# PIC4SeR/nav2_social_mpc_controller

Measured on AMD Instinct MI355X. Metric: MPC solves/sec (horizon=18, 8 agents, max 40 LM iterations, Ceres termination rules), higher is better.
Workload: dtype f64; 1 GPU; BASELINE configs[2] per GPU: batch=8192 scenes/GPU, 8 people, horizon=18 (T=28, block=6, P=6, M=226), 200x200 u8 costmap per scene, DENSE_SCHUR, max 40 LM iterations with Ceres termination rules; consecutive steps overlapped on 4 HIP streams, every stream on a scene batch of its own; scenes_per_gpu=8192, people=8, T=28, P=6, M=226, streams=4, distinct_scene_batches=4

## Files before the change

### nav2_social_mpc_controller_amd/csrc/smpc_launch.hpp

```cpp
#pragma once

#include <hip/hip_runtime.h>
#include <stdint.h>

#include "../../include/smpc.h"
#include "smpc_math.hpp"

namespace smpc {

constexpr int kWave = 64;
constexpr double kNoTarget = 1e300;
constexpr int kSoc = 15;

typedef double v4d __attribute__((ext_vector_type(4)));
typedef double v2d __attribute__((ext_vector_type(2)));

struct KParams {
  int B, T, N, CH, bl, nb, P, nbounded, nfeas;
  int size_x, size_y, costmap_shared;
  double dt, resolution;
  double inv_resolution;
  smpc_params prm;
  const double* pose0;
  const double* init_params;
  const double* path_pts;
  const double* goal_yaw;
  const double* people;
  const uint8_t* has_people;
  const int32_t* T_scene;
  const uint8_t* costmap;
  const double* costmap_origin;
  double* o_params;
  double* o_cmds;
  double* o_path;
  int32_t* o_status;
  int32_t* o_reason;
  int32_t* o_iterations;
  int32_t* o_evaluations;
  double* o_initial_cost;
  double* o_final_cost;
  int* queue;
  const double* people_rec;
  const double* people_aux;
  const int32_t* order;
  int hp_A;
  int full_gram;
  int prio_step;
  int lone_help;
  double* stage_rec;
  double* stage_aux;
  unsigned long long* stamps;
  const double* e_x;
  double* e_residuals;
  double* e_jacobian;
  double* e_cost;
  double* e_gradient;
  int e_M;
  int e_row_order;
  MathTab mt;
  AtanNodeTab an;
  const smpc_scene_params* scene_params;
  double* o_trace;
  int32_t* o_trace_n;
  int trace_rows;
  int stage_at_fetch;
};
constexpr int kTraceCols = SMPC_TRACE_COLS;
constexpr int kQueueWords = 4;

__host__ __device__ constexpr bool lone_trip_kernel(int W, bool vt, bool sp, bool trace) { return W == 32 && !vt && !sp && !trace; }

typedef const KParams __attribute__((address_space(4))) * KParamsK;

constexpr int kSensInRegsMaxBlocks = 6;
__host__ __device__ constexpr int eval_extra_doubles(int T, int P, int W) {
  return (64 / W) * (2 * T * P) + (P / 2 > kSensInRegsMaxBlocks ? (64 / W) * (5 * (P / 2) * W) : 0);
}
__host__ __device__ constexpr int atan_tab_offset(int slot_doubles, int extra_doubles) { return (slot_doubles + extra_doubles + 3) & ~3; }
constexpr int kAtanTabDoubles = kAtanNodes * kAtanNodeStride;
constexpr int kGramChunk = 16;
__host__ __device__ constexpr int gram_red_doubles(int W) { return W * (kGramChunk + 1); }
__host__ __device__ constexpr int wave_extra_doubles(int P, int W) {
  return (kWave / W) * ((P / 2 > 1 ? P / 2 - 1 : 1) * (P + 1));
}

struct LdsLayout {
  int ag;
  int valid;
  int cs;
  int inc;
  int cst;
  int stepst;
  int part;
  int hz;
  int sp;
  int lanec;
  int lm;
  int gram;
  int scratch;
  int total;
};
// ... 88 lines not shown
```

### nav2_social_mpc_controller_amd/csrc/smpc_lm.hpp

```cpp
#pragma once

#include <hip/hip_runtime.h>

#include "smpc_math.hpp"

namespace smpc {

#ifdef SMPC_STAMPS
__device__ unsigned long long g_ls_dbg[8];
#define SMPC_LS_COUNT(i, n) do { if ((threadIdx.x & 31) == 0) atomicAdd(&g_ls_dbg[i], (unsigned long long)(n)); } while (0)
#else
#define SMPC_LS_COUNT(i, n) do { } while (0)
#endif


__device__ inline void fullpiv_solve(double* A, double* b, int* perm, double* z, double* out, int n) {
  for (int i = 0; i < n; ++i) perm[i] = i;
  for (int kk = 0; kk < n; ++kk) {
    int pr = kk, pc = kk;
    double best = -1.0;
    for (int i = kk; i < n; ++i)
      for (int j = kk; j < n; ++j) {
        const double v = fabs(A[i * n + j]);
        if (v > best) { best = v; pr = i; pc = j; }
// ... 325 lines not shown
  for (int i = 0; i < 4; ++i) {
    const double rt = roots[i];
    const bool in = rt >= lo && rt <= hi;
    if (__any(in)) { const double v = eval_poly_reg<nc>(poly, rt); if (in && v < opt_v) { opt_v = v; opt_x = rt; } }
  }
  const double sx[3] = {lower.x, current.x, previous.x};
#pragma unroll
  for (int smp = 0; smp < 3; ++smp) {
    const bool in = sx[smp] >= lo && sx[smp] <= hi;
    if (__any(in)) { const double v = eval_poly_reg<nc>(poly, sx[smp]); if (in && v < opt_v) { opt_v = v; opt_x = sx[smp]; } }
  }
  step_size = opt_x;
  return true;
}

__device__ inline double clampd(double v, double lo, double hi) { return (v != v) ? v : fmin(fmax(v, lo), hi); }

__device__ inline double yaw_roundtrip(double yaw) {
  double sz, cz;
  sincos(yaw * 0.5, &sz, &cz);
  return atan2(2.0 * (cz * sz), cz * cz - sz * sz);
}


__device__ inline bool armijo_holds(double value, double cost, double gd0, double alpha) {
  return isfinite(value) && !(value > fma(1e-4 * gd0, alpha, cost));
}

enum Phase { PH_FETCH = 0, PH_INIT = 1, PH_LS = 2, PH_REEVAL = 3, PH_DONE = 4, PH_IDLE = 5 };

enum Scal { S_COST = 0, S_XNORM, S_GMAX, S_RADIUS, S_DECF, S_MCC, S_GD0, S_DIRMAX, S_PREV_X, S_PREV_V, S_PREV_G,
            S_CUR_X, S_CUR_V, S_CUR_G, S_INITIAL_COST, S_FIRST_V, S_COUNT };

struct LmRegs {
  int phase, iter, evals, num_invalid, ls_iters, n_samples, status, reason;
  bool step_successful, at_least_one, prev_vv, prev_gv, cur_vv, cur_gv, first_vv;
};

}
```

### nav2_social_mpc_controller_amd/csrc/smpc_solve_body.inc

```
  static_assert(!kSP || kVT, "a kernel with per-scene weights and bounds reads its horizon per scene as well");
  static_assert(!kTrace || (kVT && kSP), "the trace is compiled for the most general variant only");
  const auto& k = *(KParamsK)__builtin_amdgcn_kernarg_segment_ptr();
  constexpr int P = 2 * NB;
  constexpr int S = kWave / W;
  constexpr bool kLone = lone_trip_kernel(W, kVT, kSP, kTrace);
  extern __shared__ __attribute__((aligned(32))) double lds_all[];
  const int lane = threadIdx.x & 63;
  Ctx c;
  c.kp = &k;
  c.L = make_layout(Shape::T(k), Shape::N(k), P, kLayoutSolve, W, kSP);
  c.ag = k.people_rec;
  {
    double* atab = lds_all + atan_tab_offset(S * c.L.total, wave_extra_doubles(P, W));
    load_atan_nodes(c.kp, atab, lane);
    c.atab = atab;
  }
  const auto& prm = k.prm;
  const int T = Shape::T(k);
  int slot, q, qc;
  bool act;
  double *Hs, *Lw, *gs, *gu, *xc, *xt, *dl, *sc, *bc, *rs, *sv, *scratch;
  int32_t* rw;
  auto bind = [&](int lane_t) {
    slot = lane_t / W;
    c.sl = lane_t - slot * W;
    c.slot = slot;
    c.lds = lds_all + (size_t)slot * c.L.total;
    c.wave_lds = lds_all + (size_t)S * c.L.total;
    Hs = c.lds + c.L.lm;
    gs = Hs + P * P;
    gu = gs + P;
    xc = gu + P;
    xt = xc + P;
    dl = xt + P;
    sc = dl + P;
    sv = sc + P;
    rw = reinterpret_cast<int32_t*>(sv + S_COUNT);
    Lw = c.lds + c.L.cs;
    bc = Lw + P * P;
    rs = bc + 4 * P;
    scratch = rs + 3 * P;
    q = c.sl;
    act = q < P;
    qc = act ? q : 0;
  };
  bind(lane);
  auto slot_any = [&](bool pred) -> bool {
    const unsigned long long slot_bits = (W == 64) ? ~0ull : (0xffffffffull << (32 * slot));
    return (__ballot(pred) & slot_bits) != 0ull;
  };
  auto reduce3 = [&](double a, double b, double m, double& sa, double& sb, double& sm) {
    double* w3 = rs;
    if (act) { w3[q] = a; w3[P + q] = b; w3[2 * P + q] = m; }
    wave_lds_fence();
    sa = 0.0; sb = 0.0; sm = 0.0;
#pragma unroll
    for (int i = 0; i < P; ++i) { sa += w3[i]; sb += w3[P + i]; sm = fmax(sm, w3[2 * P + i]); }
  };

  auto trace_row = [&](int row, double cost, double cost_change, double gmax, double step_norm, double rho, double radius,
                       int ls_evals, bool accepted) {
    const auto& kt = *c.kp;
    if (row >= kt.trace_rows || c.sl >= kTraceCols) return;
    const int j = c.sl;
    const double v = j == 0 ? (double)row : j == 1 ? cost : j == 2 ? cost_change : j == 3 ? gmax : j == 4 ? step_norm
                   : j == 5 ? rho : j == 6 ? radius : j == 7 ? (double)ls_evals : (accepted ? 1.0 : 0.0);
    kt.o_trace[((size_t)c.scene * kt.trace_rows + row) * kTraceCols + j] = v;
  };

  LmRegs R;
  R.phase = PH_FETCH;
  R.iter = R.evals = R.num_invalid = R.ls_iters = R.n_samples = 0;
  R.status = SMPC_NO_CONVERGENCE; R.reason = SMPC_REASON_MAX_ITERATIONS;
  R.step_successful = R.at_least_one = R.prev_vv = R.prev_gv = R.cur_vv = R.cur_gv = R.first_vv = false;
  auto park = [&]() {
    rw[0] = R.iter; rw[1] = R.evals; rw[2] = R.num_invalid; rw[3] = R.ls_iters; rw[4] = R.n_samples; rw[5] = R.status;
    rw[6] = R.reason;
    rw[7] = (R.step_successful ? 1 : 0) | (R.at_least_one ? 2 : 0) | (R.prev_vv ? 4 : 0) | (R.prev_gv ? 8 : 0) |
            (R.cur_vv ? 16 : 0) | (R.cur_gv ? 32 : 0) | (R.first_vv ? 64 : 0);
  };
  auto unpark = [&]() {
    R.iter = rw[0]; R.evals = rw[1]; R.num_invalid = rw[2]; R.ls_iters = rw[3]; R.n_samples = rw[4]; R.status = rw[5];
    R.reason = rw[6];
    const int f = rw[7];
    R.step_successful = f & 1; R.at_least_one = f & 2; R.prev_vv = f & 4; R.prev_gv = f & 8;
    R.cur_vv = f & 16; R.cur_gv = f & 32; R.first_vv = f & 64;
  };
  bool ever_loaded = false;
  if constexpr (kLone) *reinterpret_cast<unsigned long long*>(rw + 8) = 0ull;
#ifdef SMPC_STAMPS
  for (int i = 0; i < 8; ++i) c.acc[i] = 0;
  for (int i = 0; i < 4; ++i) c.acc2[i] = 0;
  c.t_last = __builtin_amdgcn_s_memtime();
#endif

  for (;;) {
    SMPC_STAMP(c, 6);
    {
      KParamsK kp_t = c.kp;
      asm volatile("" : "+s"(kp_t));
      c.kp = kp_t;
    }
    const auto& k = *c.kp;
    const auto& prm = k.prm;
    const int T = Shape::T(k);
    if constexpr (!Shape::kFixed) c.L = make_layout(Shape::T(k), Shape::N(k), P, kLayoutSolve, W, kSP);
    {
      int lane_t = lane;
      asm volatile("" : "+v"(lane_t));
      bind(lane_t);
    }
    if (R.phase == PH_FETCH) {
      int scene = 0;
      if (c.sl == 0) {
        scene = atomicAdd(k.queue, 1);
        if (k.order) {
          while (scene < k.B) {
            const int want = k.order[scene];
            if (want >= 0 && want < k.B) { scene = want; break; }
            scene = atomicAdd(k.queue, 1);
          }
        }
      }
      scene = __shfl(scene, slot * W, 64);
      if (scene < k.B) {
        load_scene<W, kVT, kSP, Shape, Shape::kStageAtFetch>(c, scene);
        ever_loaded = true;
        wave_lds_fence();
        const Horizon hz0 = get_horizon<NB, kVT, Shape>(c);
        double v = 0.0;
        if (act && (q >> 1) <= hz0.blast) {
          const bool bnd = (q >> 1) < hz0.nbounded;
          const double lo0 = bnd ? ((q & 1) ? SMPC_SCENE_PRM(c, kSP, prm, w_min) : SMPC_SCENE_PRM(c, kSP, prm, v_min)) : -1.7976931348623157e308;
          const double hi0 = bnd ? ((q & 1) ? SMPC_SCENE_PRM(c, kSP, prm, w_max) : SMPC_SCENE_PRM(c, kSP, prm, v_max)) : 1.7976931348623157e308;
          v = clampd(k.init_params[(size_t)scene * P + q] + 0.0, lo0, hi0);
        }
        if (act) { xc[q] = v; xt[q] = v; }
        double xn, u0, u1;
        reduce3(v * v, 0.0, 0.0, xn, u0, u1);
        sv[S_XNORM] = fast_sqrt(xn);
        R.phase = PH_INIT;
        R.iter = 0; R.evals = 0; R.num_invalid = 0;
        R.status = SMPC_NO_CONVERGENCE; R.reason = SMPC_REASON_MAX_ITERATIONS;
        R.step_successful = true; R.at_least_one = false;
      } else {
        if (!ever_loaded) {
          load_scene<W, kVT, kSP, Shape, Shape::kStageAtFetch>(c, 0, false);
          ever_loaded = true;
          if (act) xt[q] = 0.0;
        }
        R.phase = PH_IDLE;
      }
    }
    if (__all(R.phase == PH_IDLE)) break;
    SMPC_STAMP(c, 0);
    if constexpr (kLone) {
      const bool idle = R.phase == PH_IDLE;
      const unsigned long long ib = __ballot(idle);
      const bool half = ((ib ^ (ib >> 32)) & 1ull) != 0ull;
      const bool lone = half && k.lone_help != 0 && Shape::N(k) >= 2 && __ballot(!idle && c.has_people) != 0ull;
      *trip_mode(c) = !lone ? kTripPaired : idle ? kTripHelper : kTripOwner;
      *reinterpret_cast<unsigned long long*>(rw + 8) += 1ull + (half ? 1ull << 21 : 0ull) + (lone ? 1ull << 42 : 0ull);
    }
    if (k.prio_step > 0) {
      const int mine = (R.phase == PH_IDLE) ? 0 : R.evals;
      int age = __builtin_amdgcn_readfirstlane(mine);
      if (S == 2) age = max(age, __builtin_amdgcn_readlane(mine, 32));
      const int step = k.prio_step;
      if (age >= 3 * step) __builtin_amdgcn_s_setprio(3);
      else if (age >= 2 * step) __builtin_amdgcn_s_setprio(2);
      else if (age >= step) __builtin_amdgcn_s_setprio(1);
      else __builtin_amdgcn_s_setprio(0);
    }

    park();
    const int phase_at_sweep = R.phase;
    auto need_rest = [&]() -> bool {
      if (phase_at_sweep != PH_LS) return phase_at_sweep != PH_IDLE;
      if (k.full_gram) return true;
      const double* gt = c.lds + c.L.gram;
      const double* svp = c.lds + c.L.lm + P * P + 6 * P;
      const unsigned long long slot_bits = (W == 64) ? ~0ull : (0xffffffffull << (32 * c.slot));
      const bool col_finite = (__ballot(c.sl <= P && !isfinite(gt[min(c.sl, P) * (P + 1) + P])) & slot_bits) == 0ull;
      return !col_finite || armijo_holds(0.5 * gt[P * (P + 1) + P], svp[S_COST], svp[S_GD0], svp[S_CUR_X]);
    };
    sweep<NB, W, false, kVT, kSP, Shape, kLone>(c, xt, nullptr, nullptr, need_rest);
    {
      int lane_t = lane;
      asm volatile("" : "+v"(lane_t));
      bind(lane_t);
    }
    GramView GH;
    GH.base = c.lds + c.L.gram;
    GH.ld = P + 1;
    unpark();
    const Horizon hz = get_horizon<NB, kVT, Shape>(c);
    const bool bounded = act && (q >> 1) < hz.nbounded;
    const double lo_q = bounded ? ((q & 1) ? SMPC_SCENE_PRM(c, kSP, prm, w_min) : SMPC_SCENE_PRM(c, kSP, prm, v_min)) : -1.7976931348623157e308;
    const double hi_q = bounded ? ((q & 1) ? SMPC_SCENE_PRM(c, kSP, prm, w_max) : SMPC_SCENE_PRM(c, kSP, prm, v_max)) : 1.7976931348623157e308;
    const bool gram_full = c.gram_full;
    const bool finite = !gram_full || !slot_any(c.sl <= P && !isfinite(GH.base[min(c.sl, P) * GH.ld + min(c.sl, P)]));
    const double val = 0.5 * GH(P, P);
    bool new_iteration = false;

    auto adopt_trial_point = [&]() {
      double xa = 0.0, gm = 0.0;
      if (act) {
        xa = xt[q];
        xc[q] = xa;
        const double scq = sc[q];
        const double* grow = GH.base + q * GH.ld;
#pragma unroll
        for (int b = 0; b < P; ++b) Hs[q * P + b] = grow[b] * scq * sc[b];
        const double g = grow[P];
        gu[q] = g; gs[q] = g * scq;
        gm = fabs(xa - clampd(xa - g, lo_q, hi_q));
      }
      double xn, u0, gmax;
      reduce3(xa * xa, 0.0, gm, xn, u0, gmax);
      sv[S_XNORM] = fast_sqrt(xn);
      sv[S_GMAX] = gmax;
    };
    auto candidate = [&]() {
      const double cost = sv[S_COST];
      const double cand_cost = R.cur_vv ? sv[S_CUR_V] : 1.7976931348623157e308;
      const double d = act ? xc[q] - xt[q] : 0.0;
      double sn2, u0, u1;
      reduce3(d * d, 0.0, 0.0, sn2, u0, u1);
      const double step_norm = fast_sqrt(sn2);
      const bool tol_allowed = !prm.fixed_iterations && (!prm.tol_needs_successful_step || R.at_least_one);
      if (tol_allowed && step_norm <= prm.param_tol * (sv[S_XNORM] + prm.param_tol)) {
        if constexpr (kTrace) trace_row(R.iter, cost, cost - cand_cost, sv[S_GMAX], step_norm, 0.0, sv[S_RADIUS], R.n_samples, false);
        R.status = SMPC_CONVERGENCE; R.reason = SMPC_REASON_PARAMETER_TOL; R.phase = PH_DONE; return;
      }
      const double cost_change = cost - cand_cost;
      if (tol_allowed && fabs(cost_change) <= prm.fn_tol * cost) {
        if constexpr (kTrace) trace_row(R.iter, cost, cost_change, sv[S_GMAX], step_norm, 0.0, sv[S_RADIUS], R.n_samples, false);
        R.status = SMPC_CONVERGENCE; R.reason = SMPC_REASON_FUNCTION_TOL; R.phase = PH_DONE; return;
      }
      const double rho = (cand_cost >= 1.7976931348623157e308) ? -1.7976931348623157e308 : div_fast(cost_change, sv[S_MCC]);
      if (rho > 1e-3 && !gram_full) {
        R.phase = PH_REEVAL;
        return;
      }
      if (rho > 1e-3) {
        adopt_trial_point();
        sv[S_COST] = cand_cost;
        R.step_successful = true; R.at_least_one = true;
        const double t = 2.0 * rho - 1.0;
        sv[S_RADIUS] = fmin(1e16, div_fast(sv[S_RADIUS], fmax(1.0 / 3.0, 1.0 - t * t * t)));
        sv[S_DECF] = 2.0;
      } else {
        sv[S_RADIUS] = sv[S_RADIUS] / sv[S_DECF];
        sv[S_DECF] *= 2.0;
      }
      if constexpr (kTrace) {
        trace_row(R.iter, sv[S_COST], cost_change, sv[S_GMAX], step_norm, rho, sv[S_RADIUS], R.n_samples, R.step_successful);
      }
      new_iteration = true;
    };

    if (R.phase == PH_INIT) {
      ++R.evals;
      sv[S_COST] = val;
      sv[S_INITIAL_COST] = val;
      if (kVT && reinterpret_cast<const int*>(c.lds + c.L.hz)[6] != 0) {
        R.status = SMPC_FAILURE; R.reason = SMPC_REASON_SHORT_PATH; R.phase = PH_DONE;
      } else if (!finite) {
        R.status = SMPC_FAILURE; R.reason = SMPC_REASON_EVAL_FAILED; R.phase = PH_DONE;
      } else {
        if (act) sc[q] = 1.0 / (1.0 + sqrt(GH.base[q * GH.ld + q]));
        wave_lds_fence();
        adopt_trial_point();
        sv[S_RADIUS] = 1e4; sv[S_DECF] = 2.0;
        if constexpr (kTrace) trace_row(0, val, 0.0, sv[S_GMAX], 0.0, 0.0, 1e4, 0, true);
        new_iteration = true;
      }
    } else if (R.phase == PH_LS) {
      ++R.evals;
      const double dq = act ? dl[q] : 0.0;
      double gd, u0, u1;
      reduce3(act ? dq * GH.base[q * GH.ld + P] : 0.0, 0.0, 0.0, gd, u0, u1);
      R.cur_vv = finite && isfinite(val);
      R.cur_gv = R.cur_vv && isfinite(gd);
      sv[S_CUR_V] = val; sv[S_CUR_G] = gd;
      const double alpha = sv[S_CUR_X];
      if (R.n_samples == 1) { sv[S_FIRST_V] = val; R.first_vv = R.cur_vv; }
      if (R.cur_vv && armijo_holds(val, sv[S_COST], sv[S_GD0], alpha)) {
        if (act) dl[q] = dq * alpha;
        candidate();
      } else {
        ++R.ls_iters;
        bool failed = R.ls_iters >= 20;
        double step_size = 0.0;
        if (!failed) {
          Sample lower{0.0, sv[S_COST], sv[S_GD0], true, true};
          Sample previous{sv[S_PREV_X], sv[S_PREV_V], sv[S_PREV_G], R.prev_vv, R.prev_gv};
          Sample current{alpha, val, gd, R.cur_vv, R.cur_gv};
          SMPC_STAMP(c, 6);
          if (!interpolate_step_fast(lower, previous, current, 1e-3 * alpha, 0.6 * alpha, step_size))
          { SMPC_LS_COUNT(7, 1); step_size = interpolate_step(lower, previous, current, 1e-3 * alpha, 0.6 * alpha, scratch); }
          SMPC_STAMP(c, 7);
          failed = step_size * sv[S_DIRMAX] < 1e-9;
        }
        if (!failed) {
          sv[S_PREV_X] = alpha; sv[S_PREV_V] = val; sv[S_PREV_G] = gd; R.prev_vv = R.cur_vv; R.prev_gv = R.cur_gv;
          sv[S_CUR_X] = step_size;
          if (act) xt[q] = clampd(xc[q] + step_size * dq, lo_q, hi_q);
          ++R.n_samples;
        } else if (R.n_samples > 1) {
          if (act) xt[q] = clampd(xc[q] + dq, lo_q, hi_q);
          const double v1 = R.first_vv ? sv[S_FIRST_V] : 1.7976931348623157e308;
          const bool would_accept = R.first_vv && ((sv[S_COST] - v1) / sv[S_MCC] > 1e-3);
          if (would_accept) {
            R.phase = PH_REEVAL;
          } else {
            R.cur_vv = R.first_vv;
            sv[S_CUR_V] = v1;
            wave_lds_fence();
            candidate();
          }
        } else {
          candidate();
        }
      }
    } else if (R.phase == PH_REEVAL) {
      ++R.evals;
      R.cur_vv = finite && isfinite(val);
      sv[S_CUR_V] = val;
      candidate();
    }

    if (new_iteration) {
      for (;;) {
        if (R.iter >= prm.max_iterations) { R.status = SMPC_NO_CONVERGENCE; R.reason = SMPC_REASON_MAX_ITERATIONS; R.phase = PH_DONE; break; }
        if (R.step_successful && sv[S_GMAX] <= prm.gradient_tol && !prm.fixed_iterations) { R.status = SMPC_CONVERGENCE; R.reason = SMPC_REASON_GRADIENT_TOL; R.phase = PH_DONE; break; }
        if (sv[S_RADIUS] <= 1e-32) { R.status = SMPC_CONVERGENCE; R.reason = SMPC_REASON_MIN_RADIUS; R.phase = PH_DONE; break; }
        ++R.iter;
        R.step_successful = false;
        int ql = q;
        asm volatile("" : "+v"(ql));
        const double radius = sv[S_RADIUS];
        const double inv_radius = div_fast(1.0, radius);
        double arow[P], Lr[P], invd[P];
#pragma unroll
        for (int j = 0; j < P; ++j) arow[j] = Hs[qc * P + j];
        const double gsq = act ? gs[q] : 0.0;
        const double d2 = clampd(Hs[qc * P + qc], 1e-6, 1e32) * inv_radius;
        bool ok = true;
#pragma unroll
        for (int j = 0; j < P; ++j) {
          double s_ = arow[j] + ((j == ql) ? d2 : 0.0);
#pragma unroll
          for (int kk = 0; kk < j; ++kk) s_ = fma(-Lr[kk], Lw[j * P + kk], s_);
          if (ql == j) bc[j] = s_;
          wave_lds_fence();
          const double dpiv = bc[j];
          ok = ok && (dpiv > 0.0) && isfinite(dpiv);
          const double inv = rsqrt_pos(fmax(dpiv, 1e-300));
          invd[j] = inv;
          Lr[j] = s_ * inv;
          if (act && ql > j) Lw[q * P + j] = Lr[j];
          wave_lds_fence();
        }
        double accf = gsq, yq = 0.0;
#pragma unroll
        for (int kk = 0; kk < P; ++kk) {
          const double yk_own = accf * invd[kk];
          if (ql == kk) { bc[P + kk] = yk_own; yq = yk_own; }
          wave_lds_fence();
          const double yk = bc[P + kk];
          accf = fma((ql > kk) ? -Lr[kk] : 0.0, yk, accf);
        }
        double accb = yq, zq = 0.0;
#pragma unroll
        for (int kk = P - 1; kk >= 0; --kk) {
          const double zk_own = accb * invd[kk];
          if (ql == kk) { bc[2 * P + kk] = zk_own; zq = zk_own; }
          wave_lds_fence();
          const double zk = bc[2 * P + kk];
          accb = fma((act && ql < kk) ? -Lw[kk * P + qc] : 0.0, zk, accb);
        }
        const double stepq = act ? -zq : 0.0;
        bool valid = ok && !slot_any(act && !isfinite(stepq));
        double mcc = 0.0;
        if (valid) {
          if (act) bc[3 * P + q] = stepq;
          wave_lds_fence();
          double rowv = 0.0;
#pragma unroll
          for (int b = 0; b < P; ++b) rowv = fma(arow[b], bc[3 * P + b], rowv);
          double sg, sHs, u1;
          reduce3(stepq * gsq, act ? stepq * rowv : 0.0, 0.0, sg, sHs, u1);
          mcc = -sg - 0.5 * sHs;
          valid = mcc > 0.0;
        }
        if (!valid) {
          if (++R.num_invalid >= 5) { R.status = SMPC_FAILURE; R.reason = SMPC_REASON_INVALID_STEPS; R.phase = PH_DONE; break; }
          sv[S_RADIUS] = radius / sv[S_DECF]; sv[S_DECF] *= 2.0;
          wave_lds_fence();
          if constexpr (kTrace) trace_row(R.iter, sv[S_COST], 0.0, sv[S_GMAX], 0.0, 0.0, sv[S_RADIUS], 0, false);
          continue;
        }
        R.num_invalid = 0;
        sv[S_MCC] = mcc;
        double dq = 0.0, gq = 0.0;
        if (act) {
          dq = stepq * sc[q];
          dl[q] = dq;
          gq = gu[q] * dq;
          xt[q] = clampd(xc[q] + 1.0 * dq, lo_q, hi_q);
        }
        double gd0, u0, dirmax;
        reduce3(gq, 0.0, fabs(dq), gd0, u0, dirmax);
        sv[S_GD0] = gd0; sv[S_DIRMAX] = dirmax;
        sv[S_CUR_X] = 1.0;
        R.prev_vv = R.prev_gv = false;
        R.ls_iters = 0; R.n_samples = 1;
        R.phase = PH_LS;
        break;
      }
    }

    if (R.phase == PH_DONE) {
      wave_lds_fence();
      const size_t s = c.scene;
      if (c.sl == 0) {
        if (k.o_status) k.o_status[s] = R.status;
        if (k.o_reason) k.o_reason[s] = R.reason;
        if (k.o_iterations) k.o_iterations[s] = R.iter;
        if (k.o_evaluations) k.o_evaluations[s] = R.evals;
        if (k.o_initial_cost) k.o_initial_cost[s] = sv[S_INITIAL_COST];
        if (k.o_final_cost) k.o_final_cost[s] = sv[S_COST];
        if constexpr (kTrace) {
          const bool none = R.reason == SMPC_REASON_SHORT_PATH || R.reason == SMPC_REASON_EVAL_FAILED;
          if (k.o_trace_n) k.o_trace_n[s] = none ? 0 : R.iter + (R.reason == SMPC_REASON_INVALID_STEPS ? 0 : 1);
        }
      }
      if (k.o_params && c.sl < P) k.o_params[s * P + c.sl] = xc[c.sl];
      const int Th = hz.T;
      if (k.o_cmds) {
        for (int i = c.sl; i <= T; i += W) {
          const int b = block_of_step<NB>(i, hz);
          const bool in = i <= Th;
          k.o_cmds[(s * (T + 1) + i) * 2] = in ? xc[2 * b] : 0.0;
          k.o_cmds[(s * (T + 1) + i) * 2 + 1] = in ? xc[2 * b + 1] : 0.0;
        }
      }
      if (k.o_path) {
        const double* cst = c.lds + c.L.cst;
        double yaw = wrap_angle(cst[2]);
        double my_yaw_in = yaw, my_yaw_out = yaw;
        for (int i = 0; i <= T; ++i) {
          const int b = block_of_step<NB>(i, hz);
          double nyaw;
          if constexpr (Shape::kFixed) nyaw = wrap_angle(fma(k.dt, xc[2 * b + 1], yaw));
          else nyaw = wrap_angle(yaw + xc[2 * b + 1] * k.dt);
          if (i == c.sl) { my_yaw_in = yaw; my_yaw_out = nyaw; }
          yaw = nyaw;
        }
        const int bi = block_of_step<NB>(c.sl, hz);
        double sn, cs;
        sincos(my_yaw_in, &sn, &cs);
        const double v = (c.sl <= T) ? xc[2 * bi] : 0.0;
        const double tx = v * cs * k.dt, ty = v * sn * k.dt;
        double px = cst[0], py = cst[1], mx = 0.0, my = 0.0;
        for (int i = 0; i <= T; ++i) {
          px += __shfl(tx, slot * W + i, 64);
          py += __shfl(ty, slot * W + i, 64);
          if (i == c.sl) { mx = px; my = py; }
        }
        if (c.sl <= T) {
          const bool in = c.sl <= Th;
          double* o = k.o_path + (s * (T + 1) + c.sl) * 3;
          o[0] = in ? mx : 0.0; o[1] = in ? my : 0.0; o[2] = in ? my_yaw_out : 0.0;
        }
      }
      R.phase = PH_FETCH;
    }
  }
  if constexpr (kLone) {
    const auto& ke = *c.kp;
    const LdsLayout Lx = make_layout(Shape::T(ke), Shape::N(ke), P, kLayoutSolve, W, kSP);
    if (threadIdx.x == 0) {
      const unsigned long long n = *reinterpret_cast<const unsigned long long*>(lds_all + Lx.lm + P * P + 6 * P + S_COUNT + 4);
      atomicAdd(ke.queue + 1, (int)((n >> 21) & 0x1fffffull));
      atomicAdd(ke.queue + 2, (int)(n & 0x1fffffull));
      atomicAdd(ke.queue + 3, (int)(n >> 42));
    }
  }
#ifdef SMPC_STAMPS
  if (k.stamps && lane == 0) {
    for (int i = 0; i < 8; ++i) k.stamps[(size_t)blockIdx.x * 12 + i] = c.acc[i];
    for (int i = 0; i < 4; ++i) k.stamps[(size_t)blockIdx.x * 12 + 8 + i] = c.acc2[i];
  }
#endif
```

### nav2_social_mpc_controller_amd/csrc/smpc_sweep.hpp

```cpp
#pragma once

#include <hip/hip_runtime.h>
#include <stddef.h>
#include <stdint.h>

#include "../../include/smpc.h"
#include "smpc_bicubic.hpp"
#include "smpc_launch.hpp"
#include "smpc_math.hpp"
#include "smpc_social_force.hpp"
#include "smpc_stage.hpp"

namespace smpc {

__device__ inline void wave_lds_fence() {
  __builtin_amdgcn_fence(__ATOMIC_RELEASE, "wavefront");
  __builtin_amdgcn_wave_barrier();
  __builtin_amdgcn_fence(__ATOMIC_ACQUIRE, "wavefront");
}

template <int W> __device__ inline double slot_sum(double v) {
#pragma unroll
  for (int off = W / 2; off >= 1; off >>= 1) v += __shfl_xor(v, off, 64);
  return v;
// ... 137 lines not shown
  ((kSP) ? (c).lds[(c).L.sp + offsetof(smpc_scene_params, field) / sizeof(double)] : (prm).field)

struct NeedAll { __device__ inline bool operator()() const { return true; } };
enum TripMode { kTripPaired = 0, kTripOwner = 1, kTripHelper = 2 };
__device__ inline int* trip_mode(const Ctx& c) { return reinterpret_cast<int*>(c.lds + c.L.hz) + 7; }

template <int NB, int W, bool kRows, bool kVT = false, bool kSP = false, class Shape = RuntimeShape, bool kLone = false,
          class NeedRest = NeedAll>
__device__ inline GramView sweep(Ctx& c, const double* xp, double* out_r, double* out_J, NeedRest need_rest = NeedRest()) {
  constexpr int P = 2 * NB;
  const auto& k = *c.kp;
  const int T = Shape::T(k), N = Shape::N(k), sl = c.sl;
  const Horizon hz = get_horizon<NB, kVT, Shape>(c);
  const int Th = hz.T, CH = hz.CH, bl = hz.bl;
  const double dt = k.dt;
  double* cs_ = c.lds + c.L.cs;
  double* sn_ = cs_ + (T + 1);
  const double* cst = c.lds + c.L.cst;
  const int tl = min(sl, Th - 1);
  const int myb = block_of_step<NB>(sl, hz);
  const double vb = xp[2 * myb], wb = xp[2 * myb + 1];

  const v4d* agr = reinterpret_cast<const v4d*>(c.ag) + tl;
  v4d rec0 = {0.0, 0.0, 0.0, 0.0}, rec1 = {0.0, 0.0, 0.0, 0.0};
  bool lone = false, hlp = false;
  if constexpr (kLone) {
    const int mode = *trip_mode(c);
    lone = __builtin_amdgcn_readfirstlane(mode) != kTripPaired;
    hlp = mode == kTripHelper;
  }
  if (kLone && lone) {
    const v4d* owner_agr = reinterpret_cast<const v4d*>(other_half(reinterpret_cast<unsigned long long>(agr)));
    agr = hlp ? owner_agr : agr;
    rec0 = agr[(hlp ? 1 : 0) * T]; rec1 = agr[min(hlp ? 3 : 2, N - 1) * T];
  } else
  if (c.has_people) { rec0 = agr[0]; rec1 = agr[(N > 1 ? 1 : 0) * T]; }

  double th = cst[2];
#pragma unroll
  for (int b = 0; b < NB; ++b) {
    const int start = b * bl;
    const int len = block_end(b, hz) - start;
    const int cnt = min(max(sl - start, 0), len);
    th = fma(xp[2 * b + 1] * dt, (double)cnt, th);
  }
  const double th1 = th + wb * dt;
  double* scan_ = c.lds + c.L.inc;
  const int seg_start = myb * bl;
  {
    double sn, cs;
    if (__builtin_expect(!(fabs(th) <= 1e5), 0)) sincos(th, &sn, &cs);
    else sincos_tab(&k.mt, th, &sn, &cs);
    const double fj = (double)(sl - seg_start);
    double sC = cs, sS = sn, sJC = fj * cs, sJS = fj * sn;
#pragma unroll
    for (int off = 1; off < W; off <<= 1) {
      const double uC = __shfl_up(sC, off, W), uS = __shfl_up(sS, off, W);
      const double uJC = __shfl_up(sJC, off, W), uJS = __shfl_up(sJS, off, W);
      const double m = (sl - off >= seg_start) ? 1.0 : 0.0;
      sC = fma(m, uC, sC); sS = fma(m, uS, sS); sJC = fma(m, uJC, sJC); sJS = fma(m, uJS, sJS);
    }
    if (sl <= T) {
      cs_[sl] = cs; sn_[sl] = sn;
      scan_[sl] = sC; scan_[(T + 1) + sl] = sS; scan_[2 * (T + 1) + sl] = sJC; scan_[3 * (T + 1) + sl] = sJS;
    }
  }
  wave_lds_fence();
  SMPC_STAMP(c, 1);
  double X = cst[0], Y = cst[1];
// ... 108 lines not shown
          unit_ok = t_next < Th;
          const int ts = min(t_next, Th - 1);
          cX = stp[ts]; cY = stp[T + ts]; cvx = stp[2 * T + ts]; cvy = stp[3 * T + ts]; cvm = vmask[ts];
          k_in = 0;
        } else {
          k_in += helper ? 1 : 0;
        }
        t_cur = t_next; a_cur = a_next;
      }
      wave_lds_fence();
      if (!helper && sl < Th) {
        const double* pr = part + sl * kPart;
#pragma unroll
        for (int i = 0; i < 6; ++i) soc[i] += pr[i];
#pragma unroll
        for (int i = 0; i < 4; ++i) { su[i] += pr[6 + i]; qh[i] += pr[11 + i]; }
        soc[10] += pr[10];
        const int tag = (int)pr[16];
        if (pr[15] < pbest) { pbest = pr[15]; pidx = tag & 4095; }
        redo |= tag >= 4096;
      }
    } else if constexpr (kLone) {
      double* keep = c.lds + c.L.cs + 6 * (T + 1) + 4 * sl;
      int mine = 0, step = 1;
      if (lone) {
        keep[0] = X; keep[1] = Y; keep[2] = rvx; keep[3] = rvy;
        const unsigned long long ovm = other_half(vm);
        const double oX = other_half(X), oY = other_half(Y), ovx = other_half(rvx), ovy = other_half(rvy);
        vm = hlp ? ovm : vm; X = hlp ? oX : X; Y = hlp ? oY : Y; rvx = hlp ? ovx : rvx; rvy = hlp ? ovy : rvy;
        mine = hlp ? 1 : 0;
        step = 2;
      }
      for (int a = 0; a < N; a += step) {
        const v4d rec = rec0;
        rec0 = rec1;
        const int ahead = a + mine + 2 * step;
        if (ahead < N) rec1 = agr[ahead * T];
        const double apx = rec[0], apy = rec[1], awx = rec[2], awy = rec[3];
        const double dx = X - apx, dy = Y - apy;
        double d2 = fma(dx, dx, dy * dy);
        Force F = pair_force(mt, atab, dx, dy, rvx - awx, rvy - awy);
        int special = F.special ? 1 : 0;
        {
          const bool valid = (vm >> a) & 1ull;
          SMPC_PAIR_NEAREST(d2, a, valid)
          SMPC_PAIR_ADD(F, (special != 0), d2, valid)
        }
        if (step == 2 && a + 1 < N) {
          __builtin_amdgcn_sched_barrier(0);
          F.fx = other_half(F.fx); F.fy = other_half(F.fy);
          F.dfx_dx = other_half(F.dfx_dx); F.dfy_dx = other_half(F.dfy_dx);
          F.dfx_dy = other_half(F.dfx_dy); F.dfy_dy = other_half(F.dfy_dy);
          F.dfx_dux = other_half(F.dfx_dux); F.dfy_dux = other_half(F.dfy_dux);
          F.dfx_duy = other_half(F.dfx_duy); F.dfy_duy = other_half(F.dfy_duy);
          d2 = other_half(d2);
          special = other_half(special);
          __builtin_amdgcn_sched_barrier(0);
          const bool valid = (vm >> (a + 1)) & 1ull;
          SMPC_PAIR_NEAREST(d2, (a + 1), valid)
          SMPC_PAIR_ADD(F, (special != 0), d2, valid)
        }
      }
      if (step == 2) {
        redo = redo & (mine == 0);
        X = keep[0]; Y = keep[1]; rvx = keep[2]; rvy = keep[3];
      }
    } else {
      for (int a = 0; a < N; ++a) {
        const v4d rec = rec0;
        rec0 = rec1;
        if (a + 2 < N) rec1 = agr[(a + 2) * T];
        pair(rec, a, (vm >> a) & 1ull, X, Y, rvx, rvy);
      }
    }
// ... 394 lines not shown
```

### nav2_social_mpc_controller_amd/csrc/smpc_sweep_host.hpp

```cpp
#pragma once

#include <cmath>
#include <cstdio>

#include "../../include/smpc_fixed_shapes.h"
#include "smpc_eval_kernel.hpp"
#include "smpc_host.hpp"
#include "smpc_plan.hpp"
#include "smpc_solve_kernel.hpp"
#include "smpc_stage_kernel.hpp"

namespace smpc {
__global__ void smpc_fill_scene_params_kernel(smpc_scene_params* rows, int n, const smpc_scene_params row) {
  const int i = blockIdx.x * blockDim.x + threadIdx.x;
  if (i < n) rows[i] = row;
}
}

namespace {

using smpc::Sweep;

struct Dims { int CH, bl, nb, P, M, nbounded, nfeas; };

// ... 158 lines not shown
    unsigned long long dbg[8] = {0};
    (void)hipMemcpyFromSymbol(dbg, HIP_SYMBOL(smpc::g_ls_dbg), sizeof(dbg));
    std::fprintf(stderr, "[ls counters, cumulative] root4 calls %llu trips %llu | root3 calls %llu trips %llu | cubic fits %llu quintic fits %llu "
                 "(monotone shortcut %llu) generic fallback %llu\n", dbg[0], dbg[1], dbg[2], dbg[3], dbg[4], dbg[5], dbg[6], dbg[7]);
  }
  return SMPC_OK;
}
#else
inline int stamps_attach(smpc::KParams&, int) { return SMPC_OK; }
inline int stamps_dump(smpc_handle*, const smpc::KParams&, int, bool) { return SMPC_OK; }
#endif

int launch(smpc_handle* h, Staging& st, const smpc::SweepPlan& plan, const smpc::Knobs& kn, smpc::KParams& k) {
  const bool eval = plan.kind == Sweep::Eval;
  const int S = plan.S;
  const size_t shmem = plan.shmem;
  KernelFn fn = kernel_of(plan);
  SMPC_TRY(reserve_lds(fn, shmem, "scene does not fit the 160 KiB LDS of one CU"));
  if (k.B == 0) return SMPC_OK;
  int grid = (k.B + S - 1) / S;
  if (!eval) {
    int per_cu = 0;
    SMPC_HIP_CHECK(hipOccupancyMaxActiveBlocksPerMultiprocessor(&per_cu, reinterpret_cast<const void*>(fn), smpc::kWave, shmem));
    if (h->share > 1) per_cu /= h->share;
    if (per_cu < 1) per_cu = 1;
    if (kn.max_waves_per_cu && kn.max_waves_per_cu < per_cu) per_cu = kn.max_waves_per_cu;
    if (kn.debug_grid) std::fprintf(stderr, "[smpc] solve kernel: %zu B LDS per wave, %d waves per CU\n", shmem, per_cu);
    const int resident = per_cu * h->num_cu;
    const int two_per_simd = kn.lone_waves_per_cu * h->num_cu < resident ? kn.lone_waves_per_cu * h->num_cu : resident;
    if (grid > two_per_simd) grid = (grid >= 4 * resident) ? resident : two_per_simd;
    k.queue = h->queue;
    k.full_gram = kn.full_gram ? 1 : 0;
    k.prio_step = kn.prio_step;
    k.lone_help = kn.no_lone_help ? 0 : 1;
    if (kn.debug_grid) SMPC_HIP_CHECK(hipMemsetAsync(h->queue + 1, 0, (smpc::kQueueWords - 1) * sizeof(int), h->stream));
    SMPC_HIP_CHECK(hipMemsetAsync(h->queue, 0, sizeof(int), h->stream));
  }
  SMPC_TRY(stamps_attach(k, grid));
  SMPC_TRY(st.timed([&] { hipLaunchKernelGGL(fn, dim3(grid), dim3(smpc::kWave), shmem, h->stream, k); return SMPC_OK; }));
  if (kn.debug_grid && !eval) {
    int words[smpc::kQueueWords];
    SMPC_HIP_CHECK(hipStreamSynchronize(h->stream));
    SMPC_HIP_CHECK(hipMemcpy(words, h->queue, sizeof(words), hipMemcpyDeviceToHost));
    std::fprintf(stderr, "[smpc] solve kernel: %d trips, %d with one slot idle for good, %d helped\n", words[2], words[1], words[3]);
  }
  return stamps_dump(h, k, grid, eval);
}

int check_scene_params(const smpc_scene_params* sp, size_t B) {
  for (size_t i = 0; i < B; ++i) {
    const double* v = reinterpret_cast<const double*>(sp + i);
    for (int j = 0; j < smpc::kSceneParamDoubles; ++j)
      if (!std::isfinite(v[j])) { set_error("scene_params[" + std::to_string(i) + "]: every value must be finite"); return SMPC_ERR_INVALID_ARG; }
    if (!(sp[i].v_min <= sp[i].v_max) || !(sp[i].w_min <= sp[i].w_max)) {
      set_error("scene_params[" + std::to_string(i) + "]: needs v_min <= v_max and w_min <= w_max"); return SMPC_ERR_INVALID_ARG;
    }
  }
  return SMPC_OK;
}

int neutral_rows(smpc_handle* h, smpc::KParams& k) {
  const size_t have = h->neutral_sp_bytes, need = (size_t)k.B * sizeof(smpc_scene_params);
  if (need > have) {
    SMPC_TRY(grow(&h->neutral_sp, &h->neutral_sp_bytes, need + need / 4, h->stream));
    const smpc_params& p = h->prm;
    const smpc_scene_params row = {p.distance_w, p.socialwork_w, p.velocity_w, p.angle_w, p.agent_angle_w, p.proxemics_w,
                                   p.velocity_feasibility_w, p.obstacle_w, p.goal_align_w, p.desired_linear_vel,
// ... 49 lines not shown
```

Measured before the change: 4.974 million solves/s.

## Trim LM solve overhead: split reductions, pack flags, gate trip counters, shorten agent prefetch

The three-way LDS reduction is split into specialised sum, sum-pair and sum-max variants, so unused slots are no longer written and read. The LM boolean state is packed into one flag word, which makes park and unpark a single copy. Division by the power-of-two decrease factor becomes a bit-trick reciprocal multiply. Lone-trip counting atomics are gated behind the debug flag, and the agent loop now prefetches one record ahead instead of two, which cuts register pressure but may expose more load latency.

```diff
diff --git a/nav2_social_mpc_controller_amd/csrc/smpc_launch.hpp b/nav2_social_mpc_controller_amd/csrc/smpc_launch.hpp
--- a/nav2_social_mpc_controller_amd/csrc/smpc_launch.hpp
+++ b/nav2_social_mpc_controller_amd/csrc/smpc_launch.hpp
@@ -46,7 +46,7 @@
   int hp_A;
   int full_gram;
   int prio_step;
-  int lone_help;
+  int lone_trips;
   double* stage_rec;
   double* stage_aux;
   unsigned long long* stamps;
@@ -67,6 +67,7 @@
 };
 constexpr int kTraceCols = SMPC_TRACE_COLS;
 constexpr int kQueueWords = 4;
+enum LoneTripBits { kLoneHelp = 1, kLoneCount = 2 };
 
 __host__ __device__ constexpr bool lone_trip_kernel(int W, bool vt, bool sp, bool trace) { return W == 32 && !vt && !sp && !trace; }
 
diff --git a/nav2_social_mpc_controller_amd/csrc/smpc_lm.hpp b/nav2_social_mpc_controller_amd/csrc/smpc_lm.hpp
--- a/nav2_social_mpc_controller_amd/csrc/smpc_lm.hpp
+++ b/nav2_social_mpc_controller_amd/csrc/smpc_lm.hpp
@@ -381,9 +381,19 @@
 enum Scal { S_COST = 0, S_XNORM, S_GMAX, S_RADIUS, S_DECF, S_MCC, S_GD0, S_DIRMAX, S_PREV_X, S_PREV_V, S_PREV_G,
             S_CUR_X, S_CUR_V, S_CUR_G, S_INITIAL_COST, S_FIRST_V, S_COUNT };
 
+enum LmFlag { LF_STEP_SUCCESSFUL = 1, LF_AT_LEAST_ONE = 2, LF_PREV_VV = 4, LF_PREV_GV = 8, LF_CUR_VV = 16, LF_CUR_GV = 32,
+              LF_FIRST_VV = 64 };
+
 struct LmRegs {
   int phase, iter, evals, num_invalid, ls_iters, n_samples, status, reason;
-  bool step_successful, at_least_one, prev_vv, prev_gv, cur_vv, cur_gv, first_vv;
+  int flags;
+  __device__ bool has(int f) const { return (flags & f) != 0; }
+  __device__ void set(int f, bool v) { flags = v ? (flags | f) : (flags & ~f); }
+  __device__ void copy(int to, int from) { set(to, has(from)); }
 };
 
-}
+__device__ inline double pow2_reciprocal(double d) {
+  return __longlong_as_double(0x7fe0000000000000ll - __double_as_longlong(d));
+}
+
+}
diff --git a/nav2_social_mpc_controller_amd/csrc/smpc_solve_body.inc b/nav2_social_mpc_controller_amd/csrc/smpc_solve_body.inc
--- a/nav2_social_mpc_controller_amd/csrc/smpc_solve_body.inc
+++ b/nav2_social_mpc_controller_amd/csrc/smpc_solve_body.inc
@@ -49,13 +49,33 @@
     const unsigned long long slot_bits = (W == 64) ? ~0ull : (0xffffffffull << (32 * slot));
     return (__ballot(pred) & slot_bits) != 0ull;
   };
-  auto reduce3 = [&](double a, double b, double m, double& sa, double& sb, double& sm) {
+  auto reduce_sum = [&](double a, double& sa) {
     double* w3 = rs;
-    if (act) { w3[q] = a; w3[P + q] = b; w3[2 * P + q] = m; }
+    if (act) w3[q] = a;
     wave_lds_fence();
-    sa = 0.0; sb = 0.0; sm = 0.0;
-#pragma unroll
-    for (int i = 0; i < P; ++i) { sa += w3[i]; sb += w3[P + i]; sm = fmax(sm, w3[2 * P + i]); }
+    sa = 0.0;
+#pragma unroll
+    for (int i = 0; i < P; ++i) sa += w3[i];
+  };
+  auto reduce_sum2 = [&](double a, double b, double& sa, double& sb) {
+    double* w3 = rs;
+    if (act) { w3[q] = a; w3[P + q] = b; }
+    wave_lds_fence();
+    sa = 0.0; sb = 0.0;
+#pragma unroll
+    for (int i = 0; i < P; ++i) { sa += w3[i]; sb += w3[P + i]; }
+  };
+  auto reduce_sum_max = [&](double a, double m, double& sa, double& sm) {
+    double* w3 = rs;
+    if (act) { w3[q] = a; w3[2 * P + q] = m; }
+    wave_lds_fence();
+    sa = 0.0; sm = 0.0;
+#pragma unroll
+    for (int i = 0; i < P; ++i) {
+      sa += w3[i];
+      const double mi = w3[2 * P + i];
+      asm("v_max_f64 %0, %1, %2" : "=v"(sm) : "v"(sm), "v"(mi));
+    }
   };
 
   auto trace_row = [&](int row, double cost, double cost_change, double gmax, double step_norm, double rho, double radius,
@@ -72,19 +92,14 @@
   R.phase = PH_FETCH;
   R.iter = R.evals = R.num_invalid = R.ls_iters = R.n_samples = 0;
   R.status = SMPC_NO_CONVERGENCE; R.reason = SMPC_REASON_MAX_ITERATIONS;
-  R.step_successful = R.at_least_one = R.prev_vv = R.prev_gv = R.cur_vv = R.cur_gv = R.first_vv = false;
+  R.flags = 0;
   auto park = [&]() {
     rw[0] = R.iter; rw[1] = R.evals; rw[2] = R.num_invalid; rw[3] = R.ls_iters; rw[4] = R.n_samples; rw[5] = R.status;
-    rw[6] = R.reason;
-    rw[7] = (R.step_successful ? 1 : 0) | (R.at_least_one ? 2 : 0) | (R.prev_vv ? 4 : 0) | (R.prev_gv ? 8 : 0) |
-            (R.cur_vv ? 16 : 0) | (R.cur_gv ? 32 : 0) | (R.first_vv ? 64 : 0);
+    rw[6] = R.reason; rw[7] = R.flags;
   };
   auto unpark = [&]() {
     R.iter = rw[0]; R.evals = rw[1]; R.num_invalid = rw[2]; R.ls_iters = rw[3]; R.n_samples = rw[4]; R.status = rw[5];
-    R.reason = rw[6];
-    const int f = rw[7];
-    R.step_successful = f & 1; R.at_least_one = f & 2; R.prev_vv = f & 4; R.prev_gv = f & 8;
-    R.cur_vv = f & 16; R.cur_gv = f & 32; R.first_vv = f & 64;
+    R.reason = rw[6]; R.flags = rw[7];
   };
   bool ever_loaded = false;
   if constexpr (kLone) *reinterpret_cast<unsigned long long*>(rw + 8) = 0ull;
@@ -136,13 +151,13 @@
           v = clampd(k.init_params[(size_t)scene * P + q] + 0.0, lo0, hi0);
         }
         if (act) { xc[q] = v; xt[q] = v; }
-        double xn, u0, u1;
-        reduce3(v * v, 0.0, 0.0, xn, u0, u1);
+        double xn;
+        reduce_sum(v * v, xn);
         sv[S_XNORM] = fast_sqrt(xn);
         R.phase = PH_INIT;
         R.iter = 0; R.evals = 0; R.num_invalid = 0;
         R.status = SMPC_NO_CONVERGENCE; R.reason = SMPC_REASON_MAX_ITERATIONS;
-        R.step_successful = true; R.at_least_one = false;
+        R.set(LF_STEP_SUCCESSFUL, true); R.set(LF_AT_LEAST_ONE, false);
       } else {
         if (!ever_loaded) {
           load_scene<W, kVT, kSP, Shape, Shape::kStageAtFetch>(c, 0, false);
@@ -158,9 +173,9 @@
       const bool idle = R.phase == PH_IDLE;
       const unsigned long long ib = __ballot(idle);
       const bool half = ((ib ^ (ib >> 32)) & 1ull) != 0ull;
-      const bool lone = half && k.lone_help != 0 && Shape::N(k) >= 2 && __ballot(!idle && c.has_people) != 0ull;
+      const bool lone = half && (k.lone_trips & kLoneHelp) != 0 && Shape::N(k) >= 2 && __ballot(!idle && c.has_people) != 0ull;
       *trip_mode(c) = !lone ? kTripPaired : idle ? kTripHelper : kTripOwner;
-      *reinterpret_cast<unsigned long long*>(rw + 8) += 1ull + (half ? 1ull << 21 : 0ull) + (lone ? 1ull << 42 : 0ull);
+      if (k.lone_trips & kLoneCount) *reinterpret_cast<unsigned long long*>(rw + 8) += 1ull + (half ? 1ull << 21 : 0ull) + (lone ? 1ull << 42 : 0ull);
     }
     if (k.prio_step > 0) {
       const int mine = (R.phase == PH_IDLE) ? 0 : R.evals;
@@ -216,19 +231,19 @@
         gu[q] = g; gs[q] = g * scq;
         gm = fabs(xa - clampd(xa - g, lo_q, hi_q));
       }
-      double xn, u0, gmax;
-      reduce3(xa * xa, 0.0, gm, xn, u0, gmax);
+      double xn, gmax;
+      reduce_sum_max(xa * xa, gm, xn, gmax);
       sv[S_XNORM] = fast_sqrt(xn);
       sv[S_GMAX] = gmax;
     };
     auto candidate = [&]() {
       const double cost = sv[S_COST];
-      const double cand_cost = R.cur_vv ? sv[S_CUR_V] : 1.7976931348623157e308;
+      const double cand_cost = R.has(LF_CUR_VV) ? sv[S_CUR_V] : 1.7976931348623157e308;
       const double d = act ? xc[q] - xt[q] : 0.0;
-      double sn2, u0, u1;
-      reduce3(d * d, 0.0, 0.0, sn2, u0, u1);
+      double sn2;
+      reduce_sum(d * d, sn2);
       const double step_norm = fast_sqrt(sn2);
-      const bool tol_allowed = !prm.fixed_iterations && (!prm.tol_needs_successful_step || R.at_least_one);
+      const bool tol_allowed = !prm.fixed_iterations && (!prm.tol_needs_successful_step || R.has(LF_AT_LEAST_ONE));
       if (tol_allowed && step_norm <= prm.param_tol * (sv[S_XNORM] + prm.param_tol)) {
         if constexpr (kTrace) trace_row(R.iter, cost, cost - cand_cost, sv[S_GMAX], step_norm, 0.0, sv[S_RADIUS], R.n_samples, false);
         R.status = SMPC_CONVERGENCE; R.reason = SMPC_REASON_PARAMETER_TOL; R.phase = PH_DONE; return;
@@ -246,16 +261,16 @@
       if (rho > 1e-3) {
         adopt_trial_point();
         sv[S_COST] = cand_cost;
-        R.step_successful = true; R.at_least_one = true;
+        R.flags |= LF_STEP_SUCCESSFUL | LF_AT_LEAST_ONE;
         const double t = 2.0 * rho - 1.0;
         sv[S_RADIUS] = fmin(1e16, div_fast(sv[S_RADIUS], fmax(1.0 / 3.0, 1.0 - t * t * t)));
         sv[S_DECF] = 2.0;
       } else {
-        sv[S_RADIUS] = sv[S_RADIUS] / sv[S_DECF];
+        sv[S_RADIUS] = sv[S_RADIUS] * pow2_reciprocal(sv[S_DECF]);
         sv[S_DECF] *= 2.0;
       }
       if constexpr (kTrace) {
-        trace_row(R.iter, sv[S_COST], cost_change, sv[S_GMAX], step_norm, rho, sv[S_RADIUS], R.n_samples, R.step_successful);
+        trace_row(R.iter, sv[S_COST], cost_change, sv[S_GMAX], step_norm, rho, sv[S_RADIUS], R.n_samples, R.has(LF_STEP_SUCCESSFUL));
       }
       new_iteration = true;
     };
@@ -279,14 +294,14 @@
     } else if (R.phase == PH_LS) {
       ++R.evals;
       const double dq = act ? dl[q] : 0.0;
-      double gd, u0, u1;
-      reduce3(act ? dq * GH.base[q * GH.ld + P] : 0.0, 0.0, 0.0, gd, u0, u1);
-      R.cur_vv = finite && isfinite(val);
-      R.cur_gv = R.cur_vv && isfinite(gd);
+      double gd;
+      reduce_sum(act ? dq * GH.base[q * GH.ld + P] : 0.0, gd);
+      const bool cur_vv = finite && isfinite(val), cur_gv = cur_vv && isfinite(gd);
+      R.set(LF_CUR_VV, cur_vv); R.set(LF_CUR_GV, cur_gv);
       sv[S_CUR_V] = val; sv[S_CUR_G] = gd;
       const double alpha = sv[S_CUR_X];
-      if (R.n_samples == 1) { sv[S_FIRST_V] = val; R.first_vv = R.cur_vv; }
-      if (R.cur_vv && armijo_holds(val, sv[S_COST], sv[S_GD0], alpha)) {
+      if (R.n_samples == 1) { sv[S_FIRST_V] = val; R.set(LF_FIRST_VV, cur_vv); }
+      if (cur_vv && armijo_holds(val, sv[S_COST], sv[S_GD0], alpha)) {
         if (act) dl[q] = dq * alpha;
         candidate();
       } else {
@@ -295,8 +310,8 @@
         double step_size = 0.0;
         if (!failed) {
           Sample lower{0.0, sv[S_COST], sv[S_GD0], true, true};
-          Sample previous{sv[S_PREV_X], sv[S_PREV_V], sv[S_PREV_G], R.prev_vv, R.prev_gv};
-          Sample current{alpha, val, gd, R.cur_vv, R.cur_gv};
+          Sample previous{sv[S_PREV_X], sv[S_PREV_V], sv[S_PREV_G], R.has(LF_PREV_VV), R.has(LF_PREV_GV)};
+          Sample current{alpha, val, gd, cur_vv, cur_gv};
           SMPC_STAMP(c, 6);
           if (!interpolate_step_fast(lower, previous, current, 1e-3 * alpha, 0.6 * alpha, step_size))
           { SMPC_LS_COUNT(7, 1); step_size = interpolate_step(lower, previous, current, 1e-3 * alpha, 0.6 * alpha, scratch); }
@@ -304,18 +319,18 @@
           failed = step_size * sv[S_DIRMAX] < 1e-9;
         }
         if (!failed) {
-          sv[S_PREV_X] = alpha; sv[S_PREV_V] = val; sv[S_PREV_G] = gd; R.prev_vv = R.cur_vv; R.prev_gv = R.cur_gv;
+          sv[S_PREV_X] = alpha; sv[S_PREV_V] = val; sv[S_PREV_G] = gd; R.set(LF_PREV_VV, cur_vv); R.set(LF_PREV_GV, cur_gv);
           sv[S_CUR_X] = step_size;
           if (act) xt[q] = clampd(xc[q] + step_size * dq, lo_q, hi_q);
           ++R.n_samples;
         } else if (R.n_samples > 1) {
           if (act) xt[q] = clampd(xc[q] + dq, lo_q, hi_q);
-          const double v1 = R.first_vv ? sv[S_FIRST_V] : 1.7976931348623157e308;
-          const bool would_accept = R.first_vv && ((sv[S_COST] - v1) / sv[S_MCC] > 1e-3);
+          const double v1 = R.has(LF_FIRST_VV) ? sv[S_FIRST_V] : 1.7976931348623157e308;
+          const bool would_accept = R.has(LF_FIRST_VV) && ((sv[S_COST] - v1) / sv[S_MCC] > 1e-3);
           if (would_accept) {
             R.phase = PH_REEVAL;
           } else {
-            R.cur_vv = R.first_vv;
+            R.copy(LF_CUR_VV, LF_FIRST_VV);
             sv[S_CUR_V] = v1;
             wave_lds_fence();
             candidate();
@@ -326,7 +341,7 @@
       }
     } else if (R.phase == PH_REEVAL) {
       ++R.evals;
-      R.cur_vv = finite && isfinite(val);
+      R.set(LF_CUR_VV, finite && isfinite(val));
       sv[S_CUR_V] = val;
       candidate();
     }
@@ -334,10 +349,10 @@
     if (new_iteration) {
       for (;;) {
         if (R.iter >= prm.max_iterations) { R.status = SMPC_NO_CONVERGENCE; R.reason = SMPC_REASON_MAX_ITERATIONS; R.phase = PH_DONE; break; }
-        if (R.step_successful && sv[S_GMAX] <= prm.gradient_tol && !prm.fixed_iterations) { R.status = SMPC_CONVERGENCE; R.reason = SMPC_REASON_GRADIENT_TOL; R.phase = PH_DONE; break; }
+        if (R.has(LF_STEP_SUCCESSFUL) && sv[S_GMAX] <= prm.gradient_tol && !prm.fixed_iterations) { R.status = SMPC_CONVERGENCE; R.reason = SMPC_REASON_GRADIENT_TOL; R.phase = PH_DONE; break; }
         if (sv[S_RADIUS] <= 1e-32) { R.status = SMPC_CONVERGENCE; R.reason = SMPC_REASON_MIN_RADIUS; R.phase = PH_DONE; break; }
         ++R.iter;
-        R.step_successful = false;
+        R.set(LF_STEP_SUCCESSFUL, false);
         int ql = q;
         asm volatile("" : "+v"(ql));
         const double radius = sv[S_RADIUS];
@@ -390,14 +405,14 @@
           double rowv = 0.0;
 #pragma unroll
           for (int b = 0; b < P; ++b) rowv = fma(arow[b], bc[3 * P + b], rowv);
-          double sg, sHs, u1;
-          reduce3(stepq * gsq, act ? stepq * rowv : 0.0, 0.0, sg, sHs, u1);
+          double sg, sHs;
+          reduce_sum2(stepq * gsq, act ? stepq * rowv : 0.0, sg, sHs);
           mcc = -sg - 0.5 * sHs;
           valid = mcc > 0.0;
         }
         if (!valid) {
           if (++R.num_invalid >= 5) { R.status = SMPC_FAILURE; R.reason = SMPC_REASON_INVALID_STEPS; R.phase = PH_DONE; break; }
-          sv[S_RADIUS] = radius / sv[S_DECF]; sv[S_DECF] *= 2.0;
+          sv[S_RADIUS] = radius * pow2_reciprocal(sv[S_DECF]); sv[S_DECF] *= 2.0;
           wave_lds_fence();
           if constexpr (kTrace) trace_row(R.iter, sv[S_COST], 0.0, sv[S_GMAX], 0.0, 0.0, sv[S_RADIUS], 0, false);
           continue;
@@ -411,11 +426,11 @@
           gq = gu[q] * dq;
           xt[q] = clampd(xc[q] + 1.0 * dq, lo_q, hi_q);
         }
-        double gd0, u0, dirmax;
-        reduce3(gq, 0.0, fabs(dq), gd0, u0, dirmax);
+        double gd0, dirmax;
+        reduce_sum_max(gq, fabs(dq), gd0, dirmax);
         sv[S_GD0] = gd0; sv[S_DIRMAX] = dirmax;
         sv[S_CUR_X] = 1.0;
-        R.prev_vv = R.prev_gv = false;
+        R.flags &= ~(LF_PREV_VV | LF_PREV_GV);
         R.ls_iters = 0; R.n_samples = 1;
         R.phase = PH_LS;
         break;
@@ -482,7 +497,7 @@
   if constexpr (kLone) {
     const auto& ke = *c.kp;
     const LdsLayout Lx = make_layout(Shape::T(ke), Shape::N(ke), P, kLayoutSolve, W, kSP);
-    if (threadIdx.x == 0) {
+    if ((ke.lone_trips & kLoneCount) != 0 && threadIdx.x == 0) {
       const unsigned long long n = *reinterpret_cast<const unsigned long long*>(lds_all + Lx.lm + P * P + 6 * P + S_COUNT + 4);
       atomicAdd(ke.queue + 1, (int)((n >> 21) & 0x1fffffull));
       atomicAdd(ke.queue + 2, (int)(n & 0x1fffffull));
diff --git a/nav2_social_mpc_controller_amd/csrc/smpc_sweep.hpp b/nav2_social_mpc_controller_amd/csrc/smpc_sweep.hpp
--- a/nav2_social_mpc_controller_amd/csrc/smpc_sweep.hpp
+++ b/nav2_social_mpc_controller_amd/csrc/smpc_sweep.hpp
@@ -193,9 +193,12 @@
   if (kLone && lone) {
     const v4d* owner_agr = reinterpret_cast<const v4d*>(other_half(reinterpret_cast<unsigned long long>(agr)));
     agr = hlp ? owner_agr : agr;
-    rec0 = agr[(hlp ? 1 : 0) * T]; rec1 = agr[min(hlp ? 3 : 2, N - 1) * T];
+    rec0 = agr[(hlp ? 1 : 0) * T];
   } else
-  if (c.has_people) { rec0 = agr[0]; rec1 = agr[(N > 1 ? 1 : 0) * T]; }
+  if (c.has_people) {
+    rec0 = agr[0];
+    if constexpr (!kLone) rec1 = agr[(N > 1 ? 1 : 0) * T];
+  }
 
   double th = cst[2];
 #pragma unroll
@@ -370,14 +373,11 @@
         step = 2;
       }
       for (int a = 0; a < N; a += step) {
-        const v4d rec = rec0;
-        rec0 = rec1;
-        const int ahead = a + mine + 2 * step;
-        if (ahead < N) rec1 = agr[ahead * T];
-        const double apx = rec[0], apy = rec[1], awx = rec[2], awy = rec[3];
-        const double dx = X - apx, dy = Y - apy;
+        double dx = X - rec0[0], dy = Y - rec0[1], ux = rvx - rec0[2], uy = rvy - rec0[3];
+        asm volatile("" : "+v"(dx), "+v"(dy), "+v"(ux), "+v"(uy));
+        rec0 = agr[min(a + mine + step, N - 1) * T];
         double d2 = fma(dx, dx, dy * dy);
-        Force F = pair_force(mt, atab, dx, dy, rvx - awx, rvy - awy);
+        Force F = pair_force(mt, atab, dx, dy, ux, uy);
         int special = F.special ? 1 : 0;
         {
           const bool valid = (vm >> a) & 1ull;
diff --git a/nav2_social_mpc_controller_amd/csrc/smpc_sweep_host.hpp b/nav2_social_mpc_controller_amd/csrc/smpc_sweep_host.hpp
--- a/nav2_social_mpc_controller_amd/csrc/smpc_sweep_host.hpp
+++ b/nav2_social_mpc_controller_amd/csrc/smpc_sweep_host.hpp
@@ -214,7 +214,7 @@
     k.queue = h->queue;
     k.full_gram = kn.full_gram ? 1 : 0;
     k.prio_step = kn.prio_step;
-    k.lone_help = kn.no_lone_help ? 0 : 1;
+    k.lone_trips = (kn.no_lone_help ? 0 : smpc::kLoneHelp) | (kn.debug_grid ? smpc::kLoneCount : 0);
     if (kn.debug_grid) SMPC_HIP_CHECK(hipMemsetAsync(h->queue + 1, 0, (smpc::kQueueWords - 1) * sizeof(int), h->stream));
     SMPC_HIP_CHECK(hipMemsetAsync(h->queue, 0, sizeof(int), h->stream));
   }
```

Result: faster. 5.083 million solves/s, median of 6 (+2.2%).
